# Nazukixv/LiteASR

Hardware: AMD Instinct MI355X
Metric: utterances/sec (U2-Conformer+CTC, 80-d fbank T≈1000) at 1/2/4/8 MI355X (higher is better)
Workload: dtype bf16; 1 GPU; U2-Conformer-small hybrid CTC-attention training step (fwd+loss+bwd+allreduce+clip+Noam/Adam); model=U2 enc 12x conformer d256 H4 ff2048, dec 6x, V 4233, global_batch=32, per_gpu_batch=32, seq_len=1000, label_len=40, parallelism=dp1, launch=hipgraph, ranks_seen=1, rank_launcher=env

## Files before the change

### include/liteasr_hip.h

```cpp
#ifndef LITEASR_HIP_H
#define LITEASR_HIP_H

#include <stdint.h>

#ifdef __cplusplus
extern "C" {
#endif

enum { LASR_F32 = 0, LASR_BF16 = 1, LASR_I32 = 2, LASR_I64 = 3, LASR_U8 = 4 };
enum { LASR_OK = 0, LASR_ERR_INVALID = -1, LASR_ERR_LAUNCH = -2 };
enum { LASR_ACT_NONE = 0, LASR_ACT_RELU = 1, LASR_ACT_SWISH = 2,
       LASR_ACT_GATE = 3 ,
       LASR_ACT_TANH = 4  };

const char* lasr_last_error(void);
int lasr_version(void);
int lasr_set_dropout_counter(const uint64_t* dev_counter);
int lasr_counter_add(uint64_t* dev_counter, uint64_t v, void* stream);

typedef struct lasr_gemm_args {
  int M, N, K;
  int batch, batch_div;
  const void* A; int64_t lda_m, lda_k, sa1, sa2;
  const void* B; int64_t ldb_n, ldb_k, sb1, sb2;
// ... 2 lines not shown
  int c_dtype;
  float alpha; const float* alpha_dev;
  float beta;
  const float* bias;
  int act;
  void* zout;
  const void* aux; int aux_dtype; int64_t ldaux; int aux_act;
  float drop_p; uint64_t drop_seed;
  const void* res; int res_dtype; int64_t ldres; float res_scale;
  int split_k;
  void* workspace; int64_t workspace_bytes;
  float* rowsum;
  int zout_mode;
  int tile_m, tile_n;
  int ksub;
} lasr_gemm_args;
int lasr_gemm(const lasr_gemm_args* args, void* stream);
int lasr_gemm_ln_fwd(const lasr_gemm_args* args, const float* gamma, const float* beta, float eps, void* y,
                     int y_dtype, float* mean, float* rstd, void* stream);
int lasr_gemm_ln_bwd(const lasr_gemm_args* args, const void* x, int x_dtype, const float* gamma, const float* mean,
                     const float* rstd, const void* dres, int dres_dtype, void* dx, int dx_dtype, float* part,
                     int64_t part_floats, void* gb, int gb_dtype, float bscale, float bp, uint64_t bseed,
                     void* stream);
int lasr_gemm_qbias_bwd(const lasr_gemm_args* args, const void* dqu, const void* dqv, int dt, int B, int T, int H,
                        int dk, void* dqkv, int64_t ld, float* ws, int64_t ws_floats, void* stream);
float lasr_dropout_scale(float p);
#define LASR_PLAN_GLDS 1
#define LASR_PLAN_ROWSUM_FUSED 2
#define LASR_PLAN_KSUB2 4
#define LASR_PLAN_WIDE 8
int lasr_gemm_plan(const lasr_gemm_args* args, int* tile_m, int* tile_n, int* split_k, int* flags);

int lasr_gemm_dw_group(const lasr_gemm_args* args, int n, void* stream);
int lasr_gemm_dw_group_order(int longest_first);
int lasr_gemm_narrow_tiles(int on);

typedef struct lasr_reduce_seg {
  const float* part; int64_t N; int P; int accumulate;
  float* out0; float* out1; int64_t split;
} lasr_reduce_seg;
int lasr_reduce_multi(const lasr_reduce_seg* segs, int nseg, void* stream);

int lasr_colsum(const void* X, int dtype, int64_t M, int64_t N, int64_t ldx,
                float* out, int accumulate, float* workspace, int64_t ws_floats, void* stream);

// ... 251 lines not shown
```

### liteasr_amd/_native.py

```python

from __future__ import annotations

import ctypes as C
import os

_HERE = os.path.dirname(os.path.abspath(__file__))
LIB_PATH = os.path.join(_HERE, "lib", "libliteasr_hip.so")

F32, BF16, I32, I64, U8 = 0, 1, 2, 3, 4
ACT_NONE, ACT_RELU, ACT_SWISH, ACT_GATE, ACT_TANH = 0, 1, 2, 3, 4

_p = C.c_void_p
_i = C.c_int
_l = C.c_int64
_f = C.c_float
_u = C.c_uint64


class GemmArgs(C.Structure):

    _fields_ = [
        ("M", _i), ("N", _i), ("K", _i),
        ("batch", _i), ("batch_div", _i),
        ("A", _p), ("lda_m", _l), ("lda_k", _l), ("sa1", _l), ("sa2", _l),
        ("B", _p), ("ldb_n", _l), ("ldb_k", _l), ("sb1", _l), ("sb2", _l),
        ("C", _p), ("ldc", _l), ("sc1", _l), ("sc2", _l),
        ("in_dtype", _i), ("c_dtype", _i),
        ("alpha", _f), ("alpha_dev", _p),
        ("beta", _f),
        ("bias", _p),
        ("act", _i),
        ("zout", _p),
        ("aux", _p), ("aux_dtype", _i), ("ldaux", _l), ("aux_act", _i),
        ("drop_p", _f), ("drop_seed", _u),
        ("res", _p), ("res_dtype", _i), ("ldres", _l), ("res_scale", _f),
        ("split_k", _i), ("workspace", _p), ("workspace_bytes", _l),
        ("rowsum", _p),
        ("zout_mode", _i),
        ("tile_m", _i), ("tile_n", _i), ("ksub", _i),
    ]


class Conv2Args(C.Structure):

    _fields_ = [
        ("mode", _i),
        ("B", _i), ("T1", _i), ("F1", _i), ("C", _i),
        ("y1", _p), ("w2p", _p), ("bias", _p),
        ("dy2", _p), ("dy2_rows", _l),
        ("out", _p), ("rowsum", _p),
        ("workspace", _p), ("workspace_bytes", _l),
        ("x", _p), ("T", _i), ("F", _i),
        ("dw1", _p), ("db1", _p),
    ]
# ... 190 lines not shown
```

### liteasr_amd/csrc/gemm.hip

```cpp
#include "gemm_kernel.h"
#include <algorithm>


template <bool AKC, bool BKC, typename TC>
void launch_bf16(const GemmP& p, int BM, int BN, int ks, int nw, bool glds, dim3 grid, hipStream_t st);
#define LASR_EXTERN_LAUNCH(ak, bk)                                                                         \
  extern template void launch_bf16<ak, bk, float>(const GemmP&, int, int, int, int, bool, dim3, hipStream_t); \
  extern template void launch_bf16<ak, bk, bf16_t>(const GemmP&, int, int, int, int, bool, dim3, hipStream_t);
LASR_EXTERN_LAUNCH(true, true)
LASR_EXTERN_LAUNCH(true, false)
LASR_EXTERN_LAUNCH(false, true)
LASR_EXTERN_LAUNCH(false, false)
#undef LASR_EXTERN_LAUNCH

template <typename TC>
static void dispatch(const GemmP& p, bool akc, bool bkc, int bf16in, int BM, int BN, int ks, int nw, bool glds,
                     dim3 grid, hipStream_t st) {
  if (bf16in) {
    if (akc && bkc) launch_bf16<true, true, TC>(p, BM, BN, ks, nw, glds, grid, st);
    else if (akc) launch_bf16<true, false, TC>(p, BM, BN, ks, nw, glds, grid, st);
    else if (bkc) launch_bf16<false, true, TC>(p, BM, BN, ks, nw, glds, grid, st);
    else launch_bf16<false, false, TC>(p, BM, BN, ks, nw, glds, grid, st);
  } else {
    if (akc && bkc) gemm_f32_kernel<true, true, TC><<<grid, 256, 0, st>>>(p);
    else if (akc) gemm_f32_kernel<true, false, TC><<<grid, 256, 0, st>>>(p);
    else if (bkc) gemm_f32_kernel<false, true, TC><<<grid, 256, 0, st>>>(p);
    else gemm_f32_kernel<false, false, TC><<<grid, 256, 0, st>>>(p);
  }
}

static int narrow_n_tiles = 1;
extern "C" int lasr_gemm_narrow_tiles(int on) {
  narrow_n_tiles = on != 0;
  return LASR_OK;
}

static void gemm_plan(const lasr_gemm_args* a, int* BMo, int* BNo, int* splito, int* kso = nullptr,
// ... 56 lines not shown
  *BNo = BN;
  *splito = split;
}

static bool gemm_uses_glds(const lasr_gemm_args* a) {
  if (a->in_dtype != LASR_BF16) return false;
  const bool akc = (a->lda_k == 1), bkc = (a->ldb_k == 1);
  const int64_t s_a = akc ? a->lda_m : a->lda_k;
  const int64_t s_b = bkc ? a->ldb_n : a->ldb_k;
  const bool a_vec = aligned16(a->A) && s_a % 8 == 0 && a->sa1 % 8 == 0 && a->sa2 % 8 == 0;
  const bool b_vec = aligned16(a->B) && s_b % 8 == 0 && a->sb1 % 8 == 0 && a->sb2 % 8 == 0;
  const int64_t M8 = cdiv(a->M, 8) * 8, N8 = cdiv(a->N, 8) * 8;
  return a_vec && b_vec && (akc || a->lda_k >= M8) && (bkc || a->ldb_k >= N8);
}

static bool tile_ok(int tm, int tn) {
  return (tm == 0 && tn == 0) || ((tm == 64 || tm == 128 || tm == 256) && (tn == 64 || tn == 128 || tn == 256) &&
                                  (tm < 256 || tn >= 128) && (tn < 256 || tm >= 128));
}

extern "C" int lasr_gemm_plan(const lasr_gemm_args* a, int* tile_m, int* tile_n, int* split_k, int* flags) {
  LASR_CHECK_ARG(a && tile_m && tile_n && split_k, "lasr_gemm_plan: null argument");
  int ks = 1, nw = 4;
  gemm_plan(a, tile_m, tile_n, split_k, &ks, &nw);
  const bool glds = gemm_uses_glds(a);
  if (!glds) {
    *tile_m = std::min(*tile_m, 128);
    *tile_n = std::min(*tile_n, 128);
    nw = 4;
  }
  if (flags) {
    *flags = (glds ? LASR_PLAN_GLDS : 0) | (a->rowsum && glds && a->lda_k != 1 ? LASR_PLAN_ROWSUM_FUSED : 0) |
             (glds && ks == 2 && (*tile_m < 256 || nw == 8) ? LASR_PLAN_KSUB2 : 0) |
             (glds && nw == 8 ? LASR_PLAN_WIDE : 0);
  }
  return LASR_OK;
}

extern "C" int lasr_gemm(const lasr_gemm_args* a, void* stream) { return gemm_run(a, stream, nullptr); }

int gemm_run(const lasr_gemm_args* a, void* stream, GemmRowPost* post) {
  LASR_CHECK_ARG(a != nullptr, "lasr_gemm: null args");
  LASR_CHECK_ARG(a->M >= 0 && a->N >= 0 && a->K >= 0, "lasr_gemm: negative size");
  LASR_CHECK_ARG(a->in_dtype == LASR_F32 || a->in_dtype == LASR_BF16, "lasr_gemm: bad in_dtype");
  LASR_CHECK_ARG(a->c_dtype == LASR_F32 || a->c_dtype == LASR_BF16, "lasr_gemm: bad c_dtype");
  LASR_CHECK_ARG(a->lda_m == 1 || a->lda_k == 1, "lasr_gemm: A needs a unit stride");
  LASR_CHECK_ARG(a->ldb_n == 1 || a->ldb_k == 1, "lasr_gemm: B needs a unit stride");
  LASR_CHECK_ARG(a->A && a->B && a->C, "lasr_gemm: null operand");
  LASR_CHECK_ARG(a->zout_mode == 0 || a->zout_mode == 1, "lasr_gemm: zout_mode must be 0 or 1");
  LASR_CHECK_ARG(a->act != LASR_ACT_GATE && (!a->aux || a->aux_act != LASR_ACT_NONE),
                 "lasr_gemm: act GATE is only an aux_act; aux needs an aux_act");
  LASR_CHECK_ARG(tile_ok(a->tile_m, a->tile_n) && a->ksub >= 0 && a->ksub <= 2,
                 "lasr_gemm: tile override must be 64/128/256 x 64/128/256 (256 only beside >= 128) or 0 x 0, "
                 "ksub 0, 1 or 2");
  if (a->M == 0 || a->N == 0 || a->batch == 0) return LASR_OK;
  const int batch = a->batch > 0 ? a->batch : 1;
  const int bdiv = a->batch_div > 0 ? a->batch_div : 1;
  LASR_CHECK_ARG(batch == 1 || (!a->aux && !a->res && !a->zout && !a->rowsum),
                 "lasr_gemm: aux/res/zout/rowsum only supported for batch == 1");
  LASR_CHECK_ARG(!a->rowsum || a->lda_m == 1, "lasr_gemm: rowsum needs an M-contiguous A");

  GemmP p;
  p.M = a->M; p.N = a->N; p.K = a->K; p.batch = batch; p.batch_div = bdiv;
  p.A = a->A; p.lda_m = a->lda_m; p.lda_k = a->lda_k; p.sa1 = a->sa1; p.sa2 = a->sa2;
  p.B = a->B; p.ldb_n = a->ldb_n; p.ldb_k = a->ldb_k; p.sb1 = a->sb1; p.sb2 = a->sb2;
  p.C = a->C; p.ldc = a->ldc; p.sc1 = a->sc1; p.sc2 = a->sc2;
  p.alpha = a->alpha; p.alpha_dev = a->alpha_dev; p.beta = a->beta;
  p.bias = a->bias; p.act = a->act; p.zout = a->zout; p.zout_mode = a->zout_mode;
  p.aux = a->aux; p.aux_dtype = a->aux_dtype; p.ldaux = a->ldaux; p.aux_act = a->aux_act;
// ... 37 lines not shown
  gemm_plan(a, &BM, &BN, &split, &ks, &nw);
  p.split_k = split;
  const int kstep = bf ? 32 : 16;
  p.kchunk = split > 1 ? (int)(cdiv(cdiv(a->K, split), kstep) * kstep) : a->K;
  p.ws = (float*)a->workspace;
  p.rowsum = nullptr;
  p.rs_ws = nullptr;

  hipStream_t st = (hipStream_t)stream;
  const bool glds = gemm_uses_glds(a);
  if (!glds) {
    BM = std::min(BM, 128);
    BN = std::min(BN, 128);
    nw = 4;
  }
  dim3 grid((unsigned)cdiv(a->N, BN), (unsigned)cdiv(a->M, BM), (unsigned)(batch * split));
  LASR_CHECK_ARG(grid.y <= 65535 && grid.z <= 65535, "lasr_gemm: grid too large");
  const bool rs_fused = a->rowsum && glds && !akc;
  if (rs_fused) {
    p.rowsum = a->rowsum;
    if (split > 1) p.rs_ws = p.ws + (int64_t)split * batch * a->M * a->N;
  }
  if (a->c_dtype == LASR_F32) dispatch<float>(p, akc, bkc, bf, BM, BN, ks, nw, glds, grid, st);
  else dispatch<bf16_t>(p, akc, bkc, bf, BM, BN, ks, nw, glds, grid, st);
  int rc = lasr_check_launch("lasr_gemm");
  if (!rc && split > 1 && a->split_k >= 0 && post) {
    const int r = post->launch(p, post->ctx, st);
    if (r < 0) return r;
    post->done = r;
    if (r) {
      rc = lasr_check_launch("lasr_gemm/splitk_reduce_post");
      if (rc || !a->rowsum || rs_fused) return rc;
    }
  }
  if (!rc && split > 1 && a->split_k >= 0 && !(post && post->done)) {
    const int64_t total = (int64_t)a->M * a->N * batch;
    const int nblk = (int)std::min<int64_t>(cdiv(p.v4 ? total / 4 : total, 256), 4096);
    if (a->c_dtype == LASR_F32) splitk_reduce_kernel<float><<<nblk, 256, 0, st>>>(p);
    else splitk_reduce_kernel<bf16_t><<<nblk, 256, 0, st>>>(p);
    rc = lasr_check_launch("lasr_gemm/splitk_reduce");
  }
  if (rc || !a->rowsum || rs_fused) return rc;
  const int64_t used = split > 1 ? (int64_t)split * batch * a->M * a->N : 0;
  LASR_CHECK_ARG(a->workspace && a->workspace_bytes / 4 > used, "lasr_gemm: no workspace left for the rowsum");
  return lasr_colsum(a->A, a->in_dtype, a->K, a->M, a->lda_k, a->rowsum, 1, (float*)a->workspace + used,
                     a->workspace_bytes / 4 - used, stream);
}


int launch_dw_group(const DwGroupP& g, int BM, int BN, int blocks, hipStream_t st);
static int dw_group_lpt = 1;
extern "C" int lasr_gemm_dw_group_order(int longest_first) {
  dw_group_lpt = longest_first != 0;
  return LASR_OK;
}

extern "C" int lasr_gemm_dw_group(const lasr_gemm_args* args, int n, void* stream) {
  LASR_CHECK_ARG(args && n >= 1 && n <= LASR_DW_GROUP_MAX, "lasr_gemm_dw_group: 1..%d problems", LASR_DW_GROUP_MAX);
  DwGroupP g = {};
  g.n = n;
  int ord[LASR_DW_GROUP_MAX];
  int64_t work[LASR_DW_GROUP_MAX];
  for (int i = 0; i < n; ++i) {
    const lasr_gemm_args* a = args + i;
    int bm, bn, sp, ks;
    gemm_plan(a, &bm, &bn, &sp, &ks);
    work[i] = a->split_k == 1 || sp <= 1 ? a->K : cdiv(a->K, sp);
    ord[i] = i;
  }
  if (dw_group_lpt)
    std::stable_sort(ord, ord + n, [&](int x, int y) { return work[x] > work[y]; });
  int BM0 = 0, BN0 = 0, blocks = 0;
  for (int i = 0; i < n; ++i) {
    const lasr_gemm_args* a = args + ord[i];
    LASR_CHECK_ARG(a->in_dtype == LASR_BF16 && a->c_dtype == LASR_F32, "lasr_gemm_dw_group: bf16 in, fp32 partials");
    LASR_CHECK_ARG(a->lda_m == 1 && a->lda_k != 1 && a->ldb_n == 1 && a->ldb_k != 1,
                   "lasr_gemm_dw_group: A M-contiguous and B N-contiguous (dW = dY^T X)");
    const bool direct = a->split_k == 1;
    LASR_CHECK_ARG((direct || (a->split_k < 0 && a->workspace)) && (a->batch <= 1) && a->M > 0 && a->N > 0 &&
                       a->K > 0,
                   "lasr_gemm_dw_group: partials-only problems with a workspace, or direct (split_k 1) ones");
    LASR_CHECK_ARG(!direct || (a->C && a->ldc >= a->N && (a->beta == 0.f || a->beta == 1.f) && a->alpha == 1.f &&
                               !a->alpha_dev),
                   "lasr_gemm_dw_group: a direct problem needs C, ldc >= N, beta 0 or 1, alpha 1");
    LASR_CHECK_ARG(i == 0 || direct == (g.direct[0] != 0), "lasr_gemm_dw_group: direct and split problems mixed");
    LASR_CHECK_ARG(!a->act && !a->zout && !a->aux && !a->res && a->drop_p <= 0.f && !a->bias,
                   "lasr_gemm_dw_group: no epilogue");
    LASR_CHECK_ARG(gemm_uses_glds(a), "lasr_gemm_dw_group: operands not LDS-DMA eligible");
    int BM, BN, split, ks;
// ... 17 lines not shown
    g.direct[i] = direct;
    g.C[i] = (float*)a->C; g.ldc[i] = a->ldc; g.beta[i] = a->beta; g.rowsum[i] = a->rowsum;
    g.v4[i] = a->N % 4 == 0 && aligned16(direct ? a->C : a->workspace);
    g.A[i] = a->A; g.lda[i] = a->lda_k;
    g.B[i] = a->B; g.ldb[i] = a->ldb_k;
    g.ws[i] = (float*)a->workspace;
    g.rs_ws[i] = a->rowsum && !direct ? (float*)a->workspace + (int64_t)split * a->M * a->N : nullptr;
    g.start[i] = blocks;
    const int64_t nb = cdiv(a->M, BM) * cdiv(a->N, BN) * (int64_t)split;
    LASR_CHECK_ARG(blocks + nb + 8 < (1ll << 31), "lasr_gemm_dw_group: too many blocks");
    blocks += (int)cdiv(nb, 8) * 8;
  }
  g.start[n] = blocks;
  static const int slice_xcd = [] { const char* e = getenv("LASR_DW_SLICE_XCD"); return e && e[0] ? atoi(e) : 1; }();
  g.slice_xcd = slice_xcd;
  LASR_CHECK_ARG(launch_dw_group(g, BM0, BN0, blocks, (hipStream_t)stream) == 0,
                 "lasr_gemm_dw_group: no grouped instance for tile %dx%d", BM0, BN0);
  return lasr_check_launch("lasr_gemm_dw_group");
}
```

### liteasr_amd/csrc/gemm_group.hip

```cpp
#include "gemm_kernel.h"

int launch_dw_group(const DwGroupP& g, int BM, int BN, int blocks, hipStream_t st) {
  if (BM == 64 && BN == 64) gemm_dw_group_kernel<64, 64, 3, 3><<<blocks, 256, 0, st>>>(g);
  else if (BM == 64 && BN == 128) gemm_dw_group_kernel<64, 128, 3, 2><<<blocks, 256, 0, st>>>(g);
  else if (BM == 128 && BN == 64) gemm_dw_group_kernel<128, 64, 3, 2><<<blocks, 256, 0, st>>>(g);
  else if (BM == 128 && BN == 128) gemm_dw_group_kernel<128, 128, 2, 2><<<blocks, 256, 0, st>>>(g);
  else if (BM == 256 && BN == 128) gemm_dw_group_kernel<256, 128, 3, 1, 8><<<blocks, 512, 0, st>>>(g);
  else return -1;
  return 0;
}
```

### liteasr_amd/csrc/gemm_kernel.h

```cpp
#pragma once
#include "common.h"
#include "tile.h"

#include <cstring>
#include <type_traits>

#ifndef LASR_EXP
#define LASR_EXP 0
#endif


struct ConvG {
  int B, T1, F1, T2, F2, C;
  int M2;
  int cls;
  int q32, r32;
  const bf16_t* zero;
  const float* x;
  int T0, F0;
  float* w1part;
  int w1rb;
};
typedef ConvG ConvGeom;
enum { G_LIN = 0, G_FWD = 1, G_DW = 2, G_DX = 3 };
// ... 716 lines not shown
      __builtin_amdgcn_global_load_lds((gptr_t)(base + rb + noff[i]), (lptr_t)(dst + (i * NT + wid * 64) * 8),
                                       16, 0, 0);
      f2[i] += g.r32;
      t2[i] += g.q32;
      if (f2[i] >= g.F2) { f2[i] -= g.F2; t2[i] += 1; }
      while (t2[i] >= g.T2) { t2[i] -= g.T2; b[i] += 1; }
    }
  }
};

LASR_DEV int xcd_remap(int orig, int nwg) {
  const int xcd = orig & 7, q8 = nwg >> 3, r8 = nwg & 7;
  return (xcd < r8 ? xcd * (q8 + 1) : r8 * (q8 + 1) + (xcd - r8) * q8) + (orig >> 3);
}

template <int BM, int BN, bool AKC, bool BKC, typename TC, int S, int G, int KS, int NW = 4, int EPI = EPI_RT>
LASR_DEV void gemm_glds_tile(const GemmP& p, const int tx, const int ty, const int zz) {
  static_assert(G == G_LIN || (G == G_DW ? (!AKC && !BKC) : (AKC && (G == G_FWD) == BKC)),
                "gather instance operand orientation");
  static_assert(KS == 1 || KS == 2, "k sub-tiles per ring stage");
  static_assert(NW == 4 || NW == 8, "4 waves (2 x 2) or 8 waves (2 x 4)");
  constexpr int BK = 32;
  constexpr int NT = NW * 64, WCOLS = NW / 2;
  constexpr int WM = BM / 2, WN = BN / WCOLS, FM = WM / 16, FN = WN / 16;
  constexpr int TILE = (BM + BN) * BK;
  constexpr int STAGE = KS * TILE;
  constexpr int MAIN_BYTES = S * STAGE * 2;
  constexpr int EPI_BYTES = WM * (BN + 4) * 4;
  constexpr int GL = (BM + BN) * 4 / NT;
  __shared__ __attribute__((aligned(16))) char smem_epi[MAIN_BYTES > EPI_BYTES ? MAIN_BYTES : EPI_BYTES];
  bf16_t* smem = reinterpret_cast<bf16_t*>(smem_epi);
  const int tid = threadIdx.x, lane = tid & 63, wid = tid >> 6;
  const int wr = wid / WCOLS, wc = wid % WCOLS;

  const int s = zz % p.split_k, z = zz / p.split_k;
// ... 108 lines not shown
#pragma unroll
      for (int j = 0; j < FN; ++j)
        acc[i][j] = __builtin_amdgcn_mfma_f32_16x16x32_bf16(bfr[j], af[i], acc[i][j], 0, 0, 0);
  };

  const bool do_rs = !AKC && p.rowsum != nullptr && tx == 0;
  float rs[8];
#pragma unroll
  for (int q = 0; q < 8; ++q) rs[q] = 0.f;

  const int nst = nfull / KS;
#pragma unroll
  for (int t = 0; t < S - 1; ++t)
    if (t < nst) issue(t);

  for (int kt = 0; kt < nst; ++kt) {
    const int after = min(S - 2, nst - 1 - kt);
    wait_ring<S, GL * KS>(after);
    lds_barrier();
    if (kt + S - 1 < nst) issue(kt + S - 1);
#pragma unroll
    for (int u = 0; u < KS; ++u) compute(smem + (kt % S) * STAGE + u * TILE);
    if constexpr (!AKC)
      if (do_rs)
#pragma unroll
        for (int u = 0; u < KS; ++u) rowsum_tile<BM, NT>(smem + (kt % S) * STAGE + u * TILE, tid, rs);
  }
  if constexpr (KS > 1) {
    for (int j = nst * KS; j < nfull; ++j) {
      __syncthreads();
      issue_sub(kbeg + j * BK, smem);
      wait_vmcnt<0>();
      lds_barrier();
      compute(smem);
      if constexpr (!AKC)
        if (do_rs) rowsum_tile<BM, NT>(smem, tid, rs);
    }
  }
  if (G == G_LIN && nfull < nk) {
    __syncthreads();
    TileLoader<BM, AKC, NT> la;
// ... 31 lines not shown
  }
  if constexpr (W1) {
    dx_w1_epilogue<BM, BN, NW>(p, acc, smem_epi, m0, n0, dxrow, xr);
    return;
  }
  if (p.split_k > 1) gemm_epilogue_direct<BM, BN, TC, NW>(p, acc, m0, n0, s, z, z1, z2);
  else gemm_epilogue<BM, BN, TC, true, G, NW, EPI>(p, acc, smem_epi, m0, n0, s, z, z1, z2, dxrow);
}

LASR_DEV void dw_tile_order(int wg, int nx, int ny, bool n_major, int& tx, int& ty) {
  if (n_major) { tx = wg / ny; ty = wg % ny; }
  else { tx = wg % nx; ty = wg / nx; }
}

template <int BM, int BN, bool AKC, bool BKC, typename TC, int S, int MINB = 3, int G = G_LIN, int KS = 1,
          int NW = 4, int EPI = EPI_RT>
__global__ __launch_bounds__(NW * 64, MINB * NW / 4) void gemm_bf16_glds_kernel(GemmP p) {
  const int nx = gridDim.x, ny = gridDim.y;
  const int wg = xcd_remap(blockIdx.y * nx + blockIdx.x, nx * ny);
  int tx, ty;
  dw_tile_order(wg, nx, ny, !AKC && !BKC && G == G_LIN && p.N > p.M, tx, ty);
  gemm_glds_tile<BM, BN, AKC, BKC, TC, S, G, KS, NW, EPI>(p, tx, ty, blockIdx.z);
}

#define LASR_DW_GROUP_MAX 8
struct DwGroupP {
  int n;
  int start[LASR_DW_GROUP_MAX + 1];
  int M[LASR_DW_GROUP_MAX], N[LASR_DW_GROUP_MAX], K[LASR_DW_GROUP_MAX];
  int split[LASR_DW_GROUP_MAX], kchunk[LASR_DW_GROUP_MAX], v4[LASR_DW_GROUP_MAX];
  const void* A[LASR_DW_GROUP_MAX];
  const void* B[LASR_DW_GROUP_MAX];
  int64_t lda[LASR_DW_GROUP_MAX], ldb[LASR_DW_GROUP_MAX];
  float* ws[LASR_DW_GROUP_MAX];
  float* rs_ws[LASR_DW_GROUP_MAX];
  int slice_xcd;
  int direct[LASR_DW_GROUP_MAX];
  float* C[LASR_DW_GROUP_MAX];
  int64_t ldc[LASR_DW_GROUP_MAX];
  float beta[LASR_DW_GROUP_MAX];
  float* rowsum[LASR_DW_GROUP_MAX];
};

template <int BM, int BN, int S, int MINB, int NW = 4>
__global__ __launch_bounds__(NW * 64, MINB * NW / 4) void gemm_dw_group_kernel(DwGroupP g) {
  const int blk = blockIdx.x;
  int i = 0;
  for (int j = 1; j < g.n; ++j)
    if (blk >= g.start[j]) i = j;
  const int ntx = (g.N[i] + BN - 1) / BN, nty = (g.M[i] + BM - 1) / BM, ntile = ntx * nty;
  const int local = blk - g.start[i];
  if (local >= ntile * g.split[i]) return;
  GemmP p = {};
  p.M = g.M[i]; p.N = g.N[i]; p.K = g.K[i]; p.batch = 1; p.batch_div = 1;
  p.A = g.A[i]; p.lda_m = 1; p.lda_k = g.lda[i];
  p.B = g.B[i]; p.ldb_n = 1; p.ldb_k = g.ldb[i];
  p.split_k = g.split[i]; p.kchunk = g.kchunk[i]; p.ws = g.ws[i]; p.v4 = g.v4[i];
  p.rowsum = g.rs_ws[i];
  p.rs_ws = g.rs_ws[i];
// ... 4 lines not shown
    p.c_vec = ((uintptr_t)p.C & 15) == 0 && p.ldc % 8 == 0;
    p.epi_mode = p.c_vec && p.beta == 0.f ? 0 : 2;
  }
  int tile, slice;
  const int sp = g.split[i], per = 8 / (sp > 0 ? sp : 1);
  if (g.slice_xcd && 8 % sp == 0 && ntile % per == 0 && (ntile * sp) % 8 == 0) {
    const int x = local & 7, q = local >> 3, run = ntile / per;
    slice = x / per;
    tile = (x % per) * run + q;
  } else {
    tile = xcd_remap(local % ntile, ntile);
    slice = local / ntile;
  }
  int tx, ty;
  dw_tile_order(tile, ntx, nty, p.N > p.M, tx, ty);
  gemm_glds_tile<BM, BN, false, false, float, S, G_LIN, 2, NW>(p, tx, ty, slice);
}

template <bool AKC, bool BKC, typename TC>
__global__ __launch_bounds__(256) void gemm_f32_kernel(GemmP p) {
  constexpr int BM = 64, BN = 64, BK = 16, LD = BK + 1;
  __shared__ float As[BM * LD], Bs[BN * LD];
  const int tid = threadIdx.x, lane = tid & 63, wid = tid >> 6;
  const int wr = wid >> 1, wc = wid & 1;
  const int zz = blockIdx.z;
  const int s = zz % p.split_k, z = zz / p.split_k;
  const int z1 = z / p.batch_div, z2 = z % p.batch_div;
  const float* A = (const float*)p.A + z1 * p.sa1 + z2 * p.sa2;
  const float* B = (const float*)p.B + z1 * p.sb1 + z2 * p.sb2;
  const int m0 = blockIdx.y * BM, n0 = blockIdx.x * BN;
  const int kbeg = s * p.kchunk;
// ... 124 lines not shown
  }
  if (!p.zout && p.act == LASR_ACT_NONE && !p.aux && p.drop.p <= 0.f && p.epi_mode == 0) return EPI_PLAIN;
  if (!p.zout && p.act == LASR_ACT_RELU && !p.aux && p.drop.p <= 0.f && p.epi_mode == 0) return EPI_RELU;
  if (!p.zout && p.act == LASR_ACT_NONE && p.aux && p.aux_act == LASR_ACT_RELU && p.drop.p <= 0.f && p.epi_mode == 1)
    return EPI_AUX_RELU;
  if (p.zout && p.zout_mode == 1 && p.act == LASR_ACT_SWISH && p.drop.p > 0.f && !p.aux && p.epi_mode == 0)
    return EPI_SWISH_GATE_DROP;
  if (p.zout && p.zout_mode == 1 && p.act == LASR_ACT_RELU && p.drop.p > 0.f && !p.aux && p.epi_mode == 0)
    return EPI_RELU_GATE_DROP;
  if (!p.zout && p.act == LASR_ACT_NONE && p.aux && p.aux_act == LASR_ACT_GATE && p.drop.p <= 0.f && p.epi_mode == 1)
    return EPI_AUX_GATE;
  return EPI_RT;
}

static inline bool aligned16(const void* ptr) { return ((uintptr_t)ptr & 15) == 0; }
```

### liteasr_amd/csrc/gemm_l0.hip

```cpp
#include "gemm_launch.h"

template void launch_bf16<true, true, float>(const GemmP&, int, int, int, int, bool, dim3, hipStream_t);
template void launch_bf16<true, true, bf16_t>(const GemmP&, int, int, int, int, bool, dim3, hipStream_t);
```

### liteasr_amd/csrc/gemm_l1.hip

```cpp
#include "gemm_launch.h"

template void launch_bf16<true, false, float>(const GemmP&, int, int, int, int, bool, dim3, hipStream_t);
template void launch_bf16<true, false, bf16_t>(const GemmP&, int, int, int, int, bool, dim3, hipStream_t);
```

### liteasr_amd/csrc/gemm_l2.hip

```cpp
#include "gemm_launch.h"

template void launch_bf16<false, true, float>(const GemmP&, int, int, int, int, bool, dim3, hipStream_t);
template void launch_bf16<false, true, bf16_t>(const GemmP&, int, int, int, int, bool, dim3, hipStream_t);
```

### liteasr_amd/csrc/gemm_l3.hip

```cpp
#include "gemm_launch.h"

template void launch_bf16<false, false, float>(const GemmP&, int, int, int, int, bool, dim3, hipStream_t);
template void launch_bf16<false, false, bf16_t>(const GemmP&, int, int, int, int, bool, dim3, hipStream_t);
```

### liteasr_amd/csrc/gemm_launch.h

```cpp
#pragma once
#include "gemm_kernel.h"

template <bool AKC, bool BKC, typename TC>
void launch_bf16(const GemmP& p, int BM, int BN, int ks, int nw, bool glds, dim3 grid, hipStream_t st) {
  (void)nw;
  if (glds && ks == 2 && BM < 256) {
    if (BN == 256) gemm_bf16_glds_kernel<128, 256, AKC, BKC, TC, 2, 1, G_LIN, 2><<<grid, 256, 0, st>>>(p);
    else if (BM == 128 && BN == 128) gemm_bf16_glds_kernel<128, 128, AKC, BKC, TC, 2, 2, G_LIN, 2><<<grid, 256, 0, st>>>(p);
    else if (BM == 128) gemm_bf16_glds_kernel<128, 64, AKC, BKC, TC, 3, 2, G_LIN, 2><<<grid, 256, 0, st>>>(p);
    else if (BN == 128) gemm_bf16_glds_kernel<64, 128, AKC, BKC, TC, 3, 2, G_LIN, 2><<<grid, 256, 0, st>>>(p);
    else {
      const int e = epi_code(p);
#define L64(E) gemm_bf16_glds_kernel<64, 64, AKC, BKC, TC, 3, 3, G_LIN, 2, 4, E><<<grid, 256, 0, st>>>(p)
      if constexpr (AKC && std::is_same<TC, bf16_t>::value) {
        if (e == EPI_PLAIN) { L64(EPI_PLAIN); return; }
      }
      if constexpr (AKC && !BKC && std::is_same<TC, bf16_t>::value) {
        if (e == EPI_AUX_GATE) { L64(EPI_AUX_GATE); return; }
      }
      if constexpr (AKC && BKC && std::is_same<TC, bf16_t>::value) {
        if (e == EPI_RELU_GATE_DROP) { L64(EPI_RELU_GATE_DROP); return; }
      }
#undef L64
      if constexpr (AKC && BKC && std::is_same<TC, float>::value) {
// ... 69 lines not shown
```

### liteasr_amd/csrc/tile.h

```cpp
#pragma once
#include "common.h"

typedef __bf16 bf16x8 __attribute__((ext_vector_type(8)));
typedef float f32x4 __attribute__((ext_vector_type(4)));

LASR_DEV int swz(int row) { return (0x1320 >> (((row >> 2) & 3) * 4)) & 3; }
LASR_DEV int lds_off(int row, int chunk) { return row * 32 + ((chunk ^ swz(row)) << 3); }

LASR_DEV uint4 load8(const bf16_t* src, int start, int lim, bool vec) {
  uint4 v = make_uint4(0, 0, 0, 0);
  if (vec && start + 8 <= lim) {
    v = *(const uint4*)src;
  } else {
    uint32_t e[8];
#pragma unroll
    for (int j = 0; j < 8; ++j) e[j] = (start + j < lim) ? (uint32_t)src[j] : 0u;
    v.x = e[0] | (e[1] << 16);
    v.y = e[2] | (e[3] << 16);
    v.z = e[4] | (e[5] << 16);
    v.w = e[6] | (e[7] << 16);
  }
  return v;
}

// ... 121 lines not shown
  asm volatile("ds_read_b64_tr_b16 %0, %1" : "=v"(r[1]) : "v"(tile_base + o[1]));
}
template <int R_TILE>
LASR_DEV void frag_tr_raw(const bf16_t* tile, int rbase, int lane, v2i* r) {
  const int g = lane >> 4, q = (lane >> 2) & 3, pc = (lane & 3) * 4;
  r[0] = ds_tr_asm(tile + tr_off<R_TILE>(8 * g + q, rbase + pc));
  r[1] = ds_tr_asm(tile + tr_off<R_TILE>(8 * g + 4 + q, rbase + pc));
}
typedef int v4i __attribute__((ext_vector_type(4)));
LASR_DEV v4i ds_b128_asm(const bf16_t* p) {
  v4i r;
  const uint32_t a = (uint32_t)(uintptr_t)(lptr_t)p;
  asm volatile("ds_read_b128 %0, %1" : "=v"(r) : "v"(a));
  return r;
}
template <int BM, int NT = 256>
LASR_DEV void rowsum_tile(const bf16_t* tile, int tid, float* rs) {
  constexpr int CH = BM / 8, KG = NT / CH, KR = 32 / KG;
  static_assert(KR >= 1 && KR <= 4 && KR * KG == 32, "rowsum_tile geometry");
  const int c = tid % CH, k0 = tid / CH;
  v4i r[KR];
#pragma unroll
  for (int j = 0; j < KR; ++j) r[j] = ds_b128_asm(tile + tr_off<BM>(k0 + j * KG, 8 * c));
  if constexpr (KR == 1) asm volatile("s_waitcnt lgkmcnt(0)" : "+v"(r[0]));
  else if constexpr (KR == 2) asm volatile("s_waitcnt lgkmcnt(0)" : "+v"(r[0]), "+v"(r[1]));
  else asm volatile("s_waitcnt lgkmcnt(0)" : "+v"(r[0]), "+v"(r[1]), "+v"(r[2]), "+v"(r[3]));
#pragma unroll
  for (int j = 0; j < KR; ++j)
#pragma unroll
    for (int q = 0; q < 4; ++q) {
// ... 54 lines not shown
```

### liteasr_amd/kernels.py

```python

from __future__ import annotations

import contextlib
import os
import ctypes as C
import math
from typing import Optional

import torch

from . import _native as N

_DT = {torch.float32: N.F32, torch.bfloat16: N.BF16}


def dt(t: torch.Tensor) -> int:
    try:
        return _DT[t.dtype]
    except KeyError:
        raise TypeError(f"unsupported dtype {t.dtype}") from None


def ptr(t: Optional[torch.Tensor]):
    return None if t is None else t.data_ptr()
# ... 155 lines not shown
    act: int = N.ACT_NONE,
    zout: Optional[torch.Tensor] = None,
    aux: Optional[torch.Tensor] = None,
    aux_act: int = N.ACT_NONE,
    drop_p: float = 0.0,
    drop_seed: int = 0,
    res: Optional[torch.Tensor] = None,
    res_scale: float = 1.0,
    split_k: int = 1,
    rowsum: Optional[torch.Tensor] = None,
    plan_only: bool = False,
    zout_mode: int = 0,
    group: bool = False,
    tile: Optional[tuple] = None,
    ksub: int = 0,
    ln_fwd: Optional[tuple] = None,
    ln_bwd: Optional[object] = None,
    qbias: Optional[tuple] = None,
):
    if _narrow_set[0] != GEMM_NARROW_TILES:
        N.call("lasr_gemm_narrow_tiles", int(GEMM_NARROW_TILES))
        _narrow_set[0] = GEMM_NARROW_TILES
    M, K = a.shape[-2], a.shape[-1]
    K2, Nn = b.shape[-2], b.shape[-1]
    assert K == K2 and c.shape[-2] == M and c.shape[-1] == Nn, (a.shape, b.shape, c.shape)
    assert a.dtype == b.dtype
    (sa1, sa2), (za1, za2), a_m, a_k = _split(a)
    (sb1, sb2), (zb1, zb2), b_k, b_n = _split(b)
    (sc1, sc2), (zc1, zc2), c_m, c_n = _split(c)
    assert c_n == 1, "C must be row-contiguous"
# ... 13 lines not shown
        args.lda_k = 1
    if b_k == 1 and b_n == 1:
        args.ldb_k = 1
    args.in_dtype, args.c_dtype = dt(a), dt(c)
    args.alpha, args.alpha_dev, args.beta = alpha, ptr(alpha_dev), beta
    args.bias = ptr(bias)
    args.act = act
    args.zout = ptr(zout)
    args.zout_mode = zout_mode
    if aux is not None:
        args.aux, args.aux_dtype, args.ldaux, args.aux_act = ptr(aux), dt(aux), aux.stride(0), aux_act
    args.drop_p, args.drop_seed = drop_p, drop_seed
    if tile is not None:
        args.tile_m, args.tile_n = int(tile[0]), int(tile[1])
    args.ksub = int(ksub)
    if res is not None:
        args.res, args.res_dtype, args.ldres, args.res_scale = ptr(res), dt(res), res.stride(0), res_scale
    auto_split = (split_k == 1 and SMALL_GRID_SPLIT and rowsum is None and zout is None and not group
                  and a.dtype == torch.bfloat16 and z1 * z2 == 1 and K >= 1024
                  and ((M + 63) // 64) * ((Nn + 63) // 64) < SMALL_GRID_TILES)
    if auto_split:
        split_k = 0
    args.split_k = split_k
    if rowsum is not None:
        assert rowsum.dtype == torch.float32 and rowsum.is_contiguous() and rowsum.numel() == M
        assert z1 * z2 == 1 and a_m == 1, "rowsum needs batch 1 and an M-contiguous A"
        args.rowsum = ptr(rowsum)
    if split_k != 1 or rowsum is not None:
        ns = 64 if split_k <= 0 else split_k
        need = ns * z1 * z2 * M * Nn + (ns + 128) * M if rowsum is not None else ns * z1 * z2 * M * Nn
# ... 759 lines not shown
```

Measured before the change: 3406 utterances/sec.

## Add register double-buffered pipelined k-loop for glds GEMM and grouped dW

Adds a PIPE variant of the LDS-staged bf16 GEMM main loop. It loads the MFMA fragments for one k sub-tile from LDS into registers while the MFMAs for the previous sub-tile run, and it interleaves the global-to-LDS issue between them. The goal is to hide LDS read latency behind matrix-core work. A per-call `loop` field and a compile-time plan mask pick which tile shapes use it; by default only the grouped weight-gradient kernel's 256x128 (non-64) tile path takes the new loop. The cost is higher register pressure and hand-placed waitcnt ordering, which could reduce occupancy or be fragile.

```diff
diff --git a/include/liteasr_hip.h b/include/liteasr_hip.h
--- a/include/liteasr_hip.h
+++ b/include/liteasr_hip.h
@@ -40,6 +40,7 @@
   int zout_mode;
   int tile_m, tile_n;
   int ksub;
+  int loop;
 } lasr_gemm_args;
 int lasr_gemm(const lasr_gemm_args* args, void* stream);
 int lasr_gemm_ln_fwd(const lasr_gemm_args* args, const float* gamma, const float* beta, float eps, void* y,
@@ -55,6 +56,7 @@
 #define LASR_PLAN_ROWSUM_FUSED 2
 #define LASR_PLAN_KSUB2 4
 #define LASR_PLAN_WIDE 8
+#define LASR_PLAN_PIPE 16
 int lasr_gemm_plan(const lasr_gemm_args* args, int* tile_m, int* tile_n, int* split_k, int* flags);
 
 int lasr_gemm_dw_group(const lasr_gemm_args* args, int n, void* stream);
diff --git a/liteasr_amd/_native.py b/liteasr_amd/_native.py
--- a/liteasr_amd/_native.py
+++ b/liteasr_amd/_native.py
@@ -37,7 +37,7 @@
         ("split_k", _i), ("workspace", _p), ("workspace_bytes", _l),
         ("rowsum", _p),
         ("zout_mode", _i),
-        ("tile_m", _i), ("tile_n", _i), ("ksub", _i),
+        ("tile_m", _i), ("tile_n", _i), ("ksub", _i), ("loop", _i),
     ]
 
 
diff --git a/liteasr_amd/csrc/gemm.hip b/liteasr_amd/csrc/gemm.hip
--- a/liteasr_amd/csrc/gemm.hip
+++ b/liteasr_amd/csrc/gemm.hip
@@ -3,10 +3,10 @@
 
 
 template <bool AKC, bool BKC, typename TC>
-void launch_bf16(const GemmP& p, int BM, int BN, int ks, int nw, bool glds, dim3 grid, hipStream_t st);
+void launch_bf16(const GemmP& p, int BM, int BN, int ks, int nw, bool pipe, bool glds, dim3 grid, hipStream_t st);
 #define LASR_EXTERN_LAUNCH(ak, bk)                                                                         \
-  extern template void launch_bf16<ak, bk, float>(const GemmP&, int, int, int, int, bool, dim3, hipStream_t); \
-  extern template void launch_bf16<ak, bk, bf16_t>(const GemmP&, int, int, int, int, bool, dim3, hipStream_t);
+  extern template void launch_bf16<ak, bk, float>(const GemmP&, int, int, int, int, bool, bool, dim3, hipStream_t); \
+  extern template void launch_bf16<ak, bk, bf16_t>(const GemmP&, int, int, int, int, bool, bool, dim3, hipStream_t);
 LASR_EXTERN_LAUNCH(true, true)
 LASR_EXTERN_LAUNCH(true, false)
 LASR_EXTERN_LAUNCH(false, true)
@@ -14,13 +14,13 @@
 #undef LASR_EXTERN_LAUNCH
 
 template <typename TC>
-static void dispatch(const GemmP& p, bool akc, bool bkc, int bf16in, int BM, int BN, int ks, int nw, bool glds,
-                     dim3 grid, hipStream_t st) {
+static void dispatch(const GemmP& p, bool akc, bool bkc, int bf16in, int BM, int BN, int ks, int nw, bool pipe,
+                     bool glds, dim3 grid, hipStream_t st) {
   if (bf16in) {
-    if (akc && bkc) launch_bf16<true, true, TC>(p, BM, BN, ks, nw, glds, grid, st);
-    else if (akc) launch_bf16<true, false, TC>(p, BM, BN, ks, nw, glds, grid, st);
-    else if (bkc) launch_bf16<false, true, TC>(p, BM, BN, ks, nw, glds, grid, st);
-    else launch_bf16<false, false, TC>(p, BM, BN, ks, nw, glds, grid, st);
+    if (akc && bkc) launch_bf16<true, true, TC>(p, BM, BN, ks, nw, pipe, glds, grid, st);
+    else if (akc) launch_bf16<true, false, TC>(p, BM, BN, ks, nw, pipe, glds, grid, st);
+    else if (bkc) launch_bf16<false, true, TC>(p, BM, BN, ks, nw, pipe, glds, grid, st);
+    else launch_bf16<false, false, TC>(p, BM, BN, ks, nw, pipe, glds, grid, st);
   } else {
     if (akc && bkc) gemm_f32_kernel<true, true, TC><<<grid, 256, 0, st>>>(p);
     else if (akc) gemm_f32_kernel<true, false, TC><<<grid, 256, 0, st>>>(p);
@@ -107,6 +107,15 @@
   return a_vec && b_vec && (akc || a->lda_k >= M8) && (bkc || a->ldb_k >= N8);
 }
 
+#ifndef LASR_PIPE_PLAN
+#define LASR_PIPE_PLAN 16
+#endif
+static bool gemm_pipe(const lasr_gemm_args* a, int BM, int BN, int ks) {
+  if (a->loop == 1 || !gemm_has_pipe(BM, BN, ks)) return false;
+  if (a->loop == 2) return true;
+  return (LASR_PIPE_PLAN & (BN == 256 ? 4 : BM == 128 ? 2 : 1)) != 0;
+}
+
 static bool tile_ok(int tm, int tn) {
   return (tm == 0 && tn == 0) || ((tm == 64 || tm == 128 || tm == 256) && (tn == 64 || tn == 128 || tn == 256) &&
                                   (tm < 256 || tn >= 128) && (tn < 256 || tm >= 128));
@@ -125,7 +134,8 @@
   if (flags) {
     *flags = (glds ? LASR_PLAN_GLDS : 0) | (a->rowsum && glds && a->lda_k != 1 ? LASR_PLAN_ROWSUM_FUSED : 0) |
              (glds && ks == 2 && (*tile_m < 256 || nw == 8) ? LASR_PLAN_KSUB2 : 0) |
-             (glds && nw == 8 ? LASR_PLAN_WIDE : 0);
+             (glds && nw == 8 ? LASR_PLAN_WIDE : 0) |
+             (glds && gemm_pipe(a, *tile_m, *tile_n, ks) ? LASR_PLAN_PIPE : 0);
   }
   return LASR_OK;
 }
@@ -143,9 +153,9 @@
   LASR_CHECK_ARG(a->zout_mode == 0 || a->zout_mode == 1, "lasr_gemm: zout_mode must be 0 or 1");
   LASR_CHECK_ARG(a->act != LASR_ACT_GATE && (!a->aux || a->aux_act != LASR_ACT_NONE),
                  "lasr_gemm: act GATE is only an aux_act; aux needs an aux_act");
-  LASR_CHECK_ARG(tile_ok(a->tile_m, a->tile_n) && a->ksub >= 0 && a->ksub <= 2,
+  LASR_CHECK_ARG(tile_ok(a->tile_m, a->tile_n) && a->ksub >= 0 && a->ksub <= 2 && a->loop >= 0 && a->loop <= 2,
                  "lasr_gemm: tile override must be 64/128/256 x 64/128/256 (256 only beside >= 128) or 0 x 0, "
-                 "ksub 0, 1 or 2");
+                 "ksub 0, 1 or 2, loop 0, 1 or 2");
   if (a->M == 0 || a->N == 0 || a->batch == 0) return LASR_OK;
   const int batch = a->batch > 0 ? a->batch : 1;
   const int bdiv = a->batch_div > 0 ? a->batch_div : 1;
@@ -213,6 +223,7 @@
     BN = std::min(BN, 128);
     nw = 4;
   }
+  const bool pipe = glds && gemm_pipe(a, BM, BN, ks);
   dim3 grid((unsigned)cdiv(a->N, BN), (unsigned)cdiv(a->M, BM), (unsigned)(batch * split));
   LASR_CHECK_ARG(grid.y <= 65535 && grid.z <= 65535, "lasr_gemm: grid too large");
   const bool rs_fused = a->rowsum && glds && !akc;
@@ -220,8 +231,8 @@
     p.rowsum = a->rowsum;
     if (split > 1) p.rs_ws = p.ws + (int64_t)split * batch * a->M * a->N;
   }
-  if (a->c_dtype == LASR_F32) dispatch<float>(p, akc, bkc, bf, BM, BN, ks, nw, glds, grid, st);
-  else dispatch<bf16_t>(p, akc, bkc, bf, BM, BN, ks, nw, glds, grid, st);
+  if (a->c_dtype == LASR_F32) dispatch<float>(p, akc, bkc, bf, BM, BN, ks, nw, pipe, glds, grid, st);
+  else dispatch<bf16_t>(p, akc, bkc, bf, BM, BN, ks, nw, pipe, glds, grid, st);
   int rc = lasr_check_launch("lasr_gemm");
   if (!rc && split > 1 && a->split_k >= 0 && post) {
     const int r = post->launch(p, post->ctx, st);
@@ -247,7 +258,7 @@
 }
 
 
-int launch_dw_group(const DwGroupP& g, int BM, int BN, int blocks, hipStream_t st);
+int launch_dw_group(const DwGroupP& g, int BM, int BN, bool pipe, int blocks, hipStream_t st);
 static int dw_group_lpt = 1;
 extern "C" int lasr_gemm_dw_group_order(int longest_first) {
   dw_group_lpt = longest_first != 0;
@@ -270,8 +281,11 @@
   if (dw_group_lpt)
     std::stable_sort(ord, ord + n, [&](int x, int y) { return work[x] > work[y]; });
   int BM0 = 0, BN0 = 0, blocks = 0;
+  int loop = 0;
   for (int i = 0; i < n; ++i) {
     const lasr_gemm_args* a = args + ord[i];
+    LASR_CHECK_ARG(a->loop >= 0 && a->loop <= 2, "lasr_gemm_dw_group: loop 0, 1 or 2");
+    if (a->loop && loop != 1) loop = a->loop;
     LASR_CHECK_ARG(a->in_dtype == LASR_BF16 && a->c_dtype == LASR_F32, "lasr_gemm_dw_group: bf16 in, fp32 partials");
     LASR_CHECK_ARG(a->lda_m == 1 && a->lda_k != 1 && a->ldb_n == 1 && a->ldb_k != 1,
                    "lasr_gemm_dw_group: A M-contiguous and B N-contiguous (dW = dY^T X)");
@@ -319,7 +333,8 @@
   g.start[n] = blocks;
   static const int slice_xcd = [] { const char* e = getenv("LASR_DW_SLICE_XCD"); return e && e[0] ? atoi(e) : 1; }();
   g.slice_xcd = slice_xcd;
-  LASR_CHECK_ARG(launch_dw_group(g, BM0, BN0, blocks, (hipStream_t)stream) == 0,
+  const bool pipe = loop == 2 || (loop == 0 && (LASR_PIPE_PLAN & (BM0 == 64 ? 8 : 16)) != 0);
+  LASR_CHECK_ARG(launch_dw_group(g, BM0, BN0, pipe, blocks, (hipStream_t)stream) == 0,
                  "lasr_gemm_dw_group: no grouped instance for tile %dx%d", BM0, BN0);
   return lasr_check_launch("lasr_gemm_dw_group");
 }
diff --git a/liteasr_amd/csrc/gemm_group.hip b/liteasr_amd/csrc/gemm_group.hip
--- a/liteasr_amd/csrc/gemm_group.hip
+++ b/liteasr_amd/csrc/gemm_group.hip
@@ -1,6 +1,11 @@
 #include "gemm_kernel.h"
 
-int launch_dw_group(const DwGroupP& g, int BM, int BN, int blocks, hipStream_t st) {
+int launch_dw_group(const DwGroupP& g, int BM, int BN, bool pipe, int blocks, hipStream_t st) {
+  if (pipe && dw_group_has_pipe(BM, BN)) {
+    if (BM == 64) gemm_dw_group_kernel<64, 64, 3, 3, 4, 1><<<blocks, 256, 0, st>>>(g);
+    else gemm_dw_group_kernel<256, 128, 3, 1, 8, 1><<<blocks, 512, 0, st>>>(g);
+    return 0;
+  }
   if (BM == 64 && BN == 64) gemm_dw_group_kernel<64, 64, 3, 3><<<blocks, 256, 0, st>>>(g);
   else if (BM == 64 && BN == 128) gemm_dw_group_kernel<64, 128, 3, 2><<<blocks, 256, 0, st>>>(g);
   else if (BM == 128 && BN == 64) gemm_dw_group_kernel<128, 64, 3, 2><<<blocks, 256, 0, st>>>(g);
diff --git a/liteasr_amd/csrc/gemm_kernel.h b/liteasr_amd/csrc/gemm_kernel.h
--- a/liteasr_amd/csrc/gemm_kernel.h
+++ b/liteasr_amd/csrc/gemm_kernel.h
@@ -754,11 +754,13 @@
   return (xcd < r8 ? xcd * (q8 + 1) : r8 * (q8 + 1) + (xcd - r8) * q8) + (orig >> 3);
 }
 
-template <int BM, int BN, bool AKC, bool BKC, typename TC, int S, int G, int KS, int NW = 4, int EPI = EPI_RT>
+template <int BM, int BN, bool AKC, bool BKC, typename TC, int S, int G, int KS, int NW = 4, int EPI = EPI_RT,
+          int PIPE = 0>
 LASR_DEV void gemm_glds_tile(const GemmP& p, const int tx, const int ty, const int zz) {
   static_assert(G == G_LIN || (G == G_DW ? (!AKC && !BKC) : (AKC && (G == G_FWD) == BKC)),
                 "gather instance operand orientation");
   static_assert(KS == 1 || KS == 2, "k sub-tiles per ring stage");
+  static_assert(PIPE == 0 || (PIPE == 1 && G == G_LIN && KS == 2), "pipelined loop: G_LIN with 64-deep stages");
   static_assert(NW == 4 || NW == 8, "4 waves (2 x 2) or 8 waves (2 x 4)");
   constexpr int BK = 32;
   constexpr int NT = NW * 64, WCOLS = NW / 2;
@@ -897,17 +899,82 @@
   for (int t = 0; t < S - 1; ++t)
     if (t < nst) issue(t);
 
-  for (int kt = 0; kt < nst; ++kt) {
-    const int after = min(S - 2, nst - 1 - kt);
-    wait_ring<S, GL * KS>(after);
-    lds_barrier();
-    if (kt + S - 1 < nst) issue(kt + S - 1);
-#pragma unroll
-    for (int u = 0; u < KS; ++u) compute(smem + (kt % S) * STAGE + u * TILE);
-    if constexpr (!AKC)
-      if (do_rs)
-#pragma unroll
-        for (int u = 0; u < KS; ++u) rowsum_tile<BM, NT>(smem + (kt % S) * STAGE + u * TILE, tid, rs);
+  if constexpr (PIPE == 0) {
+    for (int kt = 0; kt < nst; ++kt) {
+      const int after = min(S - 2, nst - 1 - kt);
+      wait_ring<S, GL * KS>(after);
+      lds_barrier();
+      if (kt + S - 1 < nst) issue(kt + S - 1);
+#pragma unroll
+      for (int u = 0; u < KS; ++u) compute(smem + (kt % S) * STAGE + u * TILE);
+      if constexpr (!AKC)
+        if (do_rs)
+#pragma unroll
+          for (int u = 0; u < KS; ++u) rowsum_tile<BM, NT>(smem + (kt % S) * STAGE + u * TILE, tid, rs);
+    }
+  } else {
+    constexpr int NA = AKC ? FM : 2 * FM, NB = BKC ? FN : 2 * FN, NR = NA + NB;
+    struct Frags {
+      v4i ak[AKC ? FM : 1], bk[BKC ? FN : 1];
+      v2i at[AKC ? 1 : 2 * FM], bt[BKC ? 1 : 2 * FN];
+    };
+    Frags f0, f1;
+    [[maybe_unused]] const uint32_t akoff = 2u * (uint32_t)lds_off(wr * WM + (lane & 15), lane >> 4);
+    [[maybe_unused]] const uint32_t bkoff = 2u * (uint32_t)(BM * BK + lds_off(wc * WN + (lane & 15), lane >> 4));
+    auto load_frags = [&](const bf16_t* cur, Frags& f) {
+      const uint32_t base = lds_addr(cur);
+      if constexpr (AKC) ds_b128_rows<0, FM>(base + akoff, f.ak);
+      else
+#pragma unroll
+        for (int i = 0; i < FM; ++i) frag_tr_raw_at(base, aoff[i], f.at + 2 * i);
+      if constexpr (BKC) ds_b128_rows<0, FN>(base + bkoff, f.bk);
+      else
+#pragma unroll
+        for (int j = 0; j < FN; ++j) frag_tr_raw_at(base + 2 * BM * BK, boff[j], f.bt + 2 * j);
+    };
+    auto mma = [&](Frags& f, auto after) {
+      constexpr int AFTER = decltype(after)::value;
+      wait_lgkm<AFTER>();
+      if constexpr (AKC) tie_frags<FM>(f.ak);
+      else tie_frags<2 * FM>(f.at);
+      if constexpr (BKC) tie_frags<FN>(f.bk);
+      else tie_frags<2 * FN>(f.bt);
+      bf16x8 af[FM], bfr[FN];
+#pragma unroll
+      for (int i = 0; i < FM; ++i) {
+        if constexpr (AKC) af[i] = __builtin_bit_cast(bf16x8, f.ak[i]);
+        else af[i] = frag_from_raw(f.at + 2 * i);
+      }
+#pragma unroll
+      for (int j = 0; j < FN; ++j) {
+        if constexpr (BKC) bfr[j] = __builtin_bit_cast(bf16x8, f.bk[j]);
+        else bfr[j] = frag_from_raw(f.bt + 2 * j);
+      }
+#pragma unroll
+      for (int i = 0; i < FM; ++i)
+#pragma unroll
+        for (int j = 0; j < FN; ++j)
+          acc[i][j] = __builtin_amdgcn_mfma_f32_16x16x32_bf16(bfr[j], af[i], acc[i][j], 0, 0, 0);
+    };
+    for (int kt = 0; kt < nst; ++kt) {
+      const bf16_t* cur = smem + (kt % S) * STAGE;
+      wait_ring<S, GL * KS>(min(S - 2, nst - 1 - kt));
+      lds_barrier();
+      load_frags(cur, f0);
+      if (kt > 0) mma(f1, std::integral_constant<int, NR>());
+      const bool more = kt + S - 1 < nst;
+      bf16_t* dst = smem + ((kt + S - 1) % S) * STAGE;
+      const int k0 = kbeg + (kt + S - 1) * (KS * BK);
+      if (more) issue_sub(k0, dst);
+      load_frags(cur + TILE, f1);
+      if (more) issue_sub(k0 + BK, dst + TILE);
+      mma(f0, std::integral_constant<int, NR>());
+      if constexpr (!AKC)
+        if (do_rs)
+#pragma unroll
+          for (int u = 0; u < KS; ++u) rowsum_tile<BM, NT>(cur + u * TILE, tid, rs);
+    }
+    if (nst > 0) mma(f1, std::integral_constant<int, 0>());
   }
   if constexpr (KS > 1) {
     for (int j = nst * KS; j < nfull; ++j) {
@@ -969,13 +1036,13 @@
 }
 
 template <int BM, int BN, bool AKC, bool BKC, typename TC, int S, int MINB = 3, int G = G_LIN, int KS = 1,
-          int NW = 4, int EPI = EPI_RT>
+          int NW = 4, int EPI = EPI_RT, int PIPE = 0>
 __global__ __launch_bounds__(NW * 64, MINB * NW / 4) void gemm_bf16_glds_kernel(GemmP p) {
   const int nx = gridDim.x, ny = gridDim.y;
   const int wg = xcd_remap(blockIdx.y * nx + blockIdx.x, nx * ny);
   int tx, ty;
   dw_tile_order(wg, nx, ny, !AKC && !BKC && G == G_LIN && p.N > p.M, tx, ty);
-  gemm_glds_tile<BM, BN, AKC, BKC, TC, S, G, KS, NW, EPI>(p, tx, ty, blockIdx.z);
+  gemm_glds_tile<BM, BN, AKC, BKC, TC, S, G, KS, NW, EPI, PIPE>(p, tx, ty, blockIdx.z);
 }
 
 #define LASR_DW_GROUP_MAX 8
@@ -997,7 +1064,7 @@
   float* rowsum[LASR_DW_GROUP_MAX];
 };
 
-template <int BM, int BN, int S, int MINB, int NW = 4>
+template <int BM, int BN, int S, int MINB, int NW = 4, int PIPE = 0>
 __global__ __launch_bounds__(NW * 64, MINB * NW / 4) void gemm_dw_group_kernel(DwGroupP g) {
   const int blk = blockIdx.x;
   int i = 0;
@@ -1032,7 +1099,7 @@
   }
   int tx, ty;
   dw_tile_order(tile, ntx, nty, p.N > p.M, tx, ty);
-  gemm_glds_tile<BM, BN, false, false, float, S, G_LIN, 2, NW>(p, tx, ty, slice);
+  gemm_glds_tile<BM, BN, false, false, float, S, G_LIN, 2, NW, EPI_RT, PIPE>(p, tx, ty, slice);
 }
 
 template <bool AKC, bool BKC, typename TC>
@@ -1187,3 +1254,8 @@
 }
 
 static inline bool aligned16(const void* ptr) { return ((uintptr_t)ptr & 15) == 0; }
+
+static inline bool gemm_has_pipe(int BM, int BN, int ks) {
+  return ks == 2 && ((BM == 64 && BN == 64) || (BM == 128 && BN == 64) || (BM == 128 && BN == 256));
+}
+static inline bool dw_group_has_pipe(int BM, int BN) { return (BM == 64 && BN == 64) || (BM == 256 && BN == 128); }
diff --git a/liteasr_amd/csrc/gemm_l0.hip b/liteasr_amd/csrc/gemm_l0.hip
--- a/liteasr_amd/csrc/gemm_l0.hip
+++ b/liteasr_amd/csrc/gemm_l0.hip
@@ -1,4 +1,4 @@
 #include "gemm_launch.h"
 
-template void launch_bf16<true, true, float>(const GemmP&, int, int, int, int, bool, dim3, hipStream_t);
-template void launch_bf16<true, true, bf16_t>(const GemmP&, int, int, int, int, bool, dim3, hipStream_t);
+template void launch_bf16<true, true, float>(const GemmP&, int, int, int, int, bool, bool, dim3, hipStream_t);
+template void launch_bf16<true, true, bf16_t>(const GemmP&, int, int, int, int, bool, bool, dim3, hipStream_t);
diff --git a/liteasr_amd/csrc/gemm_l1.hip b/liteasr_amd/csrc/gemm_l1.hip
--- a/liteasr_amd/csrc/gemm_l1.hip
+++ b/liteasr_amd/csrc/gemm_l1.hip
@@ -1,4 +1,4 @@
 #include "gemm_launch.h"
 
-template void launch_bf16<true, false, float>(const GemmP&, int, int, int, int, bool, dim3, hipStream_t);
-template void launch_bf16<true, false, bf16_t>(const GemmP&, int, int, int, int, bool, dim3, hipStream_t);
+template void launch_bf16<true, false, float>(const GemmP&, int, int, int, int, bool, bool, dim3, hipStream_t);
+template void launch_bf16<true, false, bf16_t>(const GemmP&, int, int, int, int, bool, bool, dim3, hipStream_t);
diff --git a/liteasr_amd/csrc/gemm_l2.hip b/liteasr_amd/csrc/gemm_l2.hip
--- a/liteasr_amd/csrc/gemm_l2.hip
+++ b/liteasr_amd/csrc/gemm_l2.hip
@@ -1,4 +1,4 @@
 #include "gemm_launch.h"
 
-template void launch_bf16<false, true, float>(const GemmP&, int, int, int, int, bool, dim3, hipStream_t);
-template void launch_bf16<false, true, bf16_t>(const GemmP&, int, int, int, int, bool, dim3, hipStream_t);
+template void launch_bf16<false, true, float>(const GemmP&, int, int, int, int, bool, bool, dim3, hipStream_t);
+template void launch_bf16<false, true, bf16_t>(const GemmP&, int, int, int, int, bool, bool, dim3, hipStream_t);
diff --git a/liteasr_amd/csrc/gemm_l3.hip b/liteasr_amd/csrc/gemm_l3.hip
--- a/liteasr_amd/csrc/gemm_l3.hip
+++ b/liteasr_amd/csrc/gemm_l3.hip
@@ -1,4 +1,4 @@
 #include "gemm_launch.h"
 
-template void launch_bf16<false, false, float>(const GemmP&, int, int, int, int, bool, dim3, hipStream_t);
-template void launch_bf16<false, false, bf16_t>(const GemmP&, int, int, int, int, bool, dim3, hipStream_t);
+template void launch_bf16<false, false, float>(const GemmP&, int, int, int, int, bool, bool, dim3, hipStream_t);
+template void launch_bf16<false, false, bf16_t>(const GemmP&, int, int, int, int, bool, bool, dim3, hipStream_t);
diff --git a/liteasr_amd/csrc/gemm_launch.h b/liteasr_amd/csrc/gemm_launch.h
--- a/liteasr_amd/csrc/gemm_launch.h
+++ b/liteasr_amd/csrc/gemm_launch.h
@@ -2,8 +2,31 @@
 #include "gemm_kernel.h"
 
 template <bool AKC, bool BKC, typename TC>
-void launch_bf16(const GemmP& p, int BM, int BN, int ks, int nw, bool glds, dim3 grid, hipStream_t st) {
+void launch_bf16(const GemmP& p, int BM, int BN, int ks, int nw, bool pipe, bool glds, dim3 grid, hipStream_t st) {
   (void)nw;
+  if (glds && pipe && gemm_has_pipe(BM, BN, ks)) {
+    if (BN == 256) gemm_bf16_glds_kernel<128, 256, AKC, BKC, TC, 2, 1, G_LIN, 2, 4, EPI_RT, 1><<<grid, 256, 0, st>>>(p);
+    else if (BM == 128) gemm_bf16_glds_kernel<128, 64, AKC, BKC, TC, 3, 2, G_LIN, 2, 4, EPI_RT, 1><<<grid, 256, 0, st>>>(p);
+    else {
+      const int e = epi_code(p);
+#define L64(E) gemm_bf16_glds_kernel<64, 64, AKC, BKC, TC, 3, 3, G_LIN, 2, 4, E, 1><<<grid, 256, 0, st>>>(p)
+      if constexpr (AKC && std::is_same<TC, bf16_t>::value) {
+        if (e == EPI_PLAIN) { L64(EPI_PLAIN); return; }
+      }
+      if constexpr (AKC && !BKC && std::is_same<TC, bf16_t>::value) {
+        if (e == EPI_AUX_GATE) { L64(EPI_AUX_GATE); return; }
+      }
+      if constexpr (AKC && BKC && std::is_same<TC, bf16_t>::value) {
+        if (e == EPI_RELU_GATE_DROP) { L64(EPI_RELU_GATE_DROP); return; }
+      }
+      if constexpr (AKC && BKC && std::is_same<TC, float>::value) {
+        if (e == EPI_RES_DROP) { L64(EPI_RES_DROP); return; }
+      }
+      L64(EPI_RT);
+#undef L64
+    }
+    return;
+  }
   if (glds && ks == 2 && BM < 256) {
     if (BN == 256) gemm_bf16_glds_kernel<128, 256, AKC, BKC, TC, 2, 1, G_LIN, 2><<<grid, 256, 0, st>>>(p);
     else if (BM == 128 && BN == 128) gemm_bf16_glds_kernel<128, 128, AKC, BKC, TC, 2, 2, G_LIN, 2><<<grid, 256, 0, st>>>(p);
diff --git a/liteasr_amd/csrc/tile.h b/liteasr_amd/csrc/tile.h
--- a/liteasr_amd/csrc/tile.h
+++ b/liteasr_amd/csrc/tile.h
@@ -159,6 +159,23 @@
   asm volatile("ds_read_b128 %0, %1" : "=v"(r) : "v"(a));
   return r;
 }
+template <int I, int N>
+LASR_DEV void ds_b128_rows(uint32_t addr, v4i* r) {
+  if constexpr (I < N) {
+    asm volatile("ds_read_b128 %0, %1 offset:%2" : "=v"(r[I]) : "v"(addr), "n"(I * 1024));
+    ds_b128_rows<I + 1, N>(addr, r);
+  }
+}
+template <int AFTER>
+LASR_DEV void wait_lgkm() {
+  asm volatile("s_waitcnt lgkmcnt(%0)" ::"n"(AFTER < 15 ? AFTER : 15));
+}
+template <int N, typename T>
+LASR_DEV void tie_frags(T* r) {
+#pragma unroll
+  for (int i = 0; i < N; ++i) asm volatile("" : "+v"(r[i]));
+}
+
 template <int BM, int NT = 256>
 LASR_DEV void rowsum_tile(const bf16_t* tile, int tid, float* rs) {
   constexpr int CH = BM / 8, KG = NT / CH, KR = 32 / KG;
diff --git a/liteasr_amd/kernels.py b/liteasr_amd/kernels.py
--- a/liteasr_amd/kernels.py
+++ b/liteasr_amd/kernels.py
@@ -193,6 +193,7 @@
     group: bool = False,
     tile: Optional[tuple] = None,
     ksub: int = 0,
+    loop: int = 0,
     ln_fwd: Optional[tuple] = None,
     ln_bwd: Optional[object] = None,
     qbias: Optional[tuple] = None,
@@ -236,6 +237,7 @@
     if tile is not None:
         args.tile_m, args.tile_n = int(tile[0]), int(tile[1])
     args.ksub = int(ksub)
+    args.loop = int(loop)
     if res is not None:
         args.res, args.res_dtype, args.ldres, args.res_scale = ptr(res), dt(res), res.stride(0), res_scale
     auto_split = (split_k == 1 and SMALL_GRID_SPLIT and rowsum is None and zout is None and not group
```

Result: no change. 3420 utterances/sec, median of 6 (+0.4%).
